# templeblock/audioSignalProcess

Measured on AMD Instinct MI355X. Metric: audio frames/sec (10 ms @16 kHz) Wiener NS, higher is better.
Workload: dtype f32

## Files before the change

audiosignalprocess_amd/csrc/ns_device.h:

```cpp
#pragma once
#include <hip/hip_runtime.h>

namespace aspns_dev {

#ifdef NS1_BUDGET
#define ASP_NS_RARE(c) (__builtin_assume(!(c)), false)
#else
#define ASP_NS_RARE(c) __builtin_expect((c), 0)
#endif

__device__ __forceinline__ float xorf(float x, uint32_t m) {
  return __uint_as_float(__float_as_uint(x) ^ m);
}

__device__ __forceinline__ void wave_lds_fence() {
  __builtin_amdgcn_fence(__ATOMIC_RELEASE, "wavefront");
  __builtin_amdgcn_wave_barrier();
  __builtin_amdgcn_fence(__ATOMIC_ACQUIRE, "wavefront");
}

template <int CTRL>
__device__ __forceinline__ float dpp_move(float v) {
  return __int_as_float(__builtin_amdgcn_update_dpp(0, __float_as_int(v), CTRL, 0xF, 0xF, true));
}
// ... 223 lines not shown
  __device__ __forceinline__ float get(int k) const { return k == 0 ? a.x : k == 1 ? a.y : k == 2 ? b.x : k == 3 ? b.y : t; }
};
__device__ __forceinline__ F5 operator+(const F5& x, const F5& y) { return F5(x.a + y.a, x.b + y.b, x.t + y.t); }
__device__ __forceinline__ F5 operator-(const F5& x, const F5& y) { return F5(x.a - y.a, x.b - y.b, x.t - y.t); }
__device__ __forceinline__ F5 operator*(const F5& x, const F5& y) { return F5(x.a * y.a, x.b * y.b, x.t * y.t); }
__device__ __forceinline__ F5 operator*(float c, const F5& y) { return F5(c) * y; }
__device__ __forceinline__ F5 operator*(const F5& x, float c) { return x * F5(c); }
__device__ __forceinline__ F5 operator+(const F5& x, float c) { return x + F5(c); }
__device__ __forceinline__ F5 operator-(const F5& x, float c) { return x - F5(c); }
__device__ __forceinline__ F5 operator-(float c, const F5& y) { return F5(c) - y; }
__device__ __forceinline__ F5 operator-(const F5& x) { return F5(-x.a, -x.b, -x.t); }
__device__ __forceinline__ F5 fma5(const F5& x, const F5& y, const F5& z) {
  return F5(__builtin_elementwise_fma(x.a, y.a, z.a), __builtin_elementwise_fma(x.b, y.b, z.b),
            __builtin_fmaf(x.t, y.t, z.t));
}
__device__ __forceinline__ F5 abs5(const F5& x) {
  return F5(f32x2{fabsf(x.a.x), fabsf(x.a.y)}, f32x2{fabsf(x.b.x), fabsf(x.b.y)}, fabsf(x.t));
}
#define ASP_F5_CMP(name, op)                                                        \
  __device__ __forceinline__ B5 name(const F5& x, const F5& y) {                    \
    B5 r;                                                                           \
    r.v[0] = x.a.x op y.a.x; r.v[1] = x.a.y op y.a.y; r.v[2] = x.b.x op y.b.x;      \
    r.v[3] = x.b.y op y.b.y; r.v[4] = x.t op y.t;                                   \
    return r;                                                                       \
  }
ASP_F5_CMP(gt5, >)
ASP_F5_CMP(lt5, <)
#undef ASP_F5_CMP
__device__ __forceinline__ F5 sel5(const B5& c, const F5& x, const F5& y) {
  return F5(f32x2{c.v[0] ? x.a.x : y.a.x, c.v[1] ? x.a.y : y.a.y},
            f32x2{c.v[2] ? x.b.x : y.b.x, c.v[3] ? x.b.y : y.b.y}, c.v[4] ? x.t : y.t);
}
__device__ __forceinline__ F5 div_by_uniform5(const F5& a, float d, float rd) {
  const F5 q0 = a * rd;
  const F5 r = fma5(F5(-d), q0, a);
  return fma5(r, F5(rd), q0);
}
__device__ __forceinline__ F5 fdiv5v(const F5& n, const F5& d) {
  return F5(fdiv2(n.a, d.a), fdiv2(n.b, d.b), fdiv(n.t, d.t));
}

__device__ __forceinline__ double log_lean_f64(float x) {
  const int xb = __float_as_int(x);
  int e = ((xb >> 23) & 0xff) - 127;
  float mf = __int_as_float((xb & 0x007fffff) | 0x3f800000);
  const bool big = mf > 1.41421356f;
  mf = big ? mf * 0.5f : mf;
  e += big ? 1 : 0;
  const float ff = mf - 1.0f;
  const float gf = mf + 1.0f;
  const double g = (double)mf + 1.0;
  const double c = (double)__builtin_amdgcn_rcpf(gf);
  const double f = (double)ff;
  const double s0 = f * c;
  const double d = __builtin_fma(g, c, -1.0);
  double s = __builtin_fma(-s0, d, s0);
  s = __builtin_fma(s0 * d, d, s);
  const double z = s * s;
  double p = 2.0 / 21.0;
  p = __builtin_fma(p, z, 2.0 / 19.0);
  p = __builtin_fma(p, z, 2.0 / 17.0);
  p = __builtin_fma(p, z, 2.0 / 15.0);
  p = __builtin_fma(p, z, 2.0 / 13.0);
  p = __builtin_fma(p, z, 2.0 / 11.0);
  p = __builtin_fma(p, z, 2.0 / 9.0);
  p = __builtin_fma(p, z, 2.0 / 7.0);
  p = __builtin_fma(p, z, 2.0 / 5.0);
  p = __builtin_fma(p, z, 2.0 / 3.0);
  const double lm = __builtin_fma(s * z, p, s + s);
  const double ed = (double)e;
  const double ln2_hi = 0x1.62e42fefa38p-1;
  const double ln2_lo = 0x1.ef35793c7673p-45;
  return __builtin_fma(ed, ln2_hi, __builtin_fma(ed, ln2_lo, lm));
}

__device__ __forceinline__ bool f64_rounds_safely_to_f32(double y) {
  const unsigned lo = (unsigned)__double2loint(y) & 0x1fffffffu;
  return ((lo - 0x0ffffe00u) > 0x400u);
}
__device__ __forceinline__ bool f64_lo_rounds_unsafely(unsigned lo) { return ((lo << 3) - 0x7ffff000u) <= 0x2000u; }
__device__ __forceinline__ bool f64_rounds_unsafely_to_f32(double y) {
  return f64_lo_rounds_unsafely((unsigned)__double2loint(y));
}

__device__ __forceinline__ double exp_lean_f64(float xf, const double* __restrict__ t64) {
  const double x = (double)xf;
  const double kd = __builtin_rint(x * 0x1.71547652b82fep+6);
  const int k = (int)kd;
  double r = __builtin_fma(-kd, 0x1.62e42ff000000p-7, x);
  r = __builtin_fma(-kd, -0x1.718432a1b0e26p-41, r);
  double q = 1.0 / 120.0;
  q = __builtin_fma(q, r, 1.0 / 24.0);
  q = __builtin_fma(q, r, 1.0 / 6.0);
  q = __builtin_fma(q, r, 0.5);
  const double p = __builtin_fma(q, r * r, r);
  const double T = t64[k & 63];
  return __builtin_amdgcn_ldexp(__builtin_fma(T, p, T), k >> 6);
}

__device__ __forceinline__ float exp_f32_via_f64(float x, const double* __restrict__ t64) {
  const bool in_range = fabsf(x) <= 87.0f;
  const double y = exp_lean_f64(in_range ? x : 0.0f, t64);
  const bool ok = in_range && f64_rounds_safely_to_f32(y);
  float r = (float)y;
  if (ASP_NS_RARE(!ok)) r = (float)exp((double)x);
  return r;
}

__device__ __forceinline__ float tanh_f32_via_f64(float a, const double* __restrict__ t64) {
  const float ax = fabsf(a);
  const bool finite_ok = ax <= 40.0f;
  const double ad = (double)ax;
  const double a2 = ad * ad;
  double sr = 0x1.664f4882c10fap-6;
  sr = __builtin_fma(sr, a2, -0x1.ba1ba1ba1ba1cp-5);
  sr = __builtin_fma(sr, a2, 0x1.1111111111111p-3);
  sr = __builtin_fma(sr, a2, -0x1.5555555555555p-2);
  const double t_small = __builtin_fma(ad * a2, sr, ad);
  const double u = exp_lean_f64(finite_ok ? -2.0f * ax : 0.0f, t64);
  const double num = 1.0 - u, den = 1.0 + u;
  double rc = (double)__builtin_amdgcn_rcpf((float)den);
  rc = __builtin_fma(__builtin_fma(-den, rc, 1.0), rc, rc);
  rc = __builtin_fma(__builtin_fma(-den, rc, 1.0), rc, rc);
  double qv = num * rc;
  qv = __builtin_fma(__builtin_fma(-qv, den, num), rc, qv);
  const double t = ax < 0.03125f ? t_small : qv;
  const bool ok = finite_ok && f64_rounds_safely_to_f32(t);
  float r = __builtin_copysignf((float)t, a);
  if (ASP_NS_RARE(!ok)) r = (float)tanh((double)a);
  return r;
}

__device__ __forceinline__ float tanh_f32_via_f64_wave(float a, const double* __restrict__ t64) {
  const float ax = fabsf(a);
  const unsigned long long far = __builtin_amdgcn_ballot_w64(!(ax <= 40.0f));
  const double u = exp_lean_f64(-2.0f * ax, t64);
  const double num = 1.0 - u, den = 1.0 + u;
  double rc = (double)__builtin_amdgcn_rcpf((float)den);
  rc = __builtin_fma(__builtin_fma(-den, rc, 1.0), rc, rc);
  double t = num * rc;
  t = __builtin_fma(__builtin_fma(-t, den, num), rc, t);
  const bool small = ax < 0.03125f;
  if (ASP_NS_RARE(__builtin_amdgcn_ballot_w64(small) != 0)) {
    const double ad = (double)ax;
    const double a2 = ad * ad;
    double sr = 0x1.664f4882c10fap-6;
    sr = __builtin_fma(sr, a2, -0x1.ba1ba1ba1ba1cp-5);
    sr = __builtin_fma(sr, a2, 0x1.1111111111111p-3);
    sr = __builtin_fma(sr, a2, -0x1.5555555555555p-2);
    const double t_small = __builtin_fma(ad * a2, sr, ad);
    t = small ? t_small : t;
  }
  const unsigned long long bad = far | __builtin_amdgcn_ballot_w64(f64_rounds_unsafely_to_f32(t));
  float r = __builtin_copysignf((float)t, a);
  if (ASP_NS_RARE(bad != 0)) r = (float)tanh((double)a);
  return r;
}

__device__ __forceinline__ float fsqrt(float x) {
  const float r = __builtin_amdgcn_rsqf(x);
  float g = x * r;
  float h = 0.5f * r;
  const float e = __builtin_fmaf(-h, g, 0.5f);
  g = __builtin_fmaf(g, e, g);
  h = __builtin_fmaf(h, e, h);
  const float d = __builtin_fmaf(-g, g, x);
// ... 16 lines not shown
constexpr unsigned kLogOff = 0x3f328000u;
__device__ __forceinline__ unsigned log_reduced_bits_mad(int k, unsigned ix) {
  unsigned z;
  asm("v_mad_i32_i24 %0, %1, %2, %3" : "=v"(z) : "v"(k), "s"(0xff800000u), "v"(ix));
  return z;
}
template <bool MAD = false>
__device__ __forceinline__ double log_tab_f64(float x, const double2* __restrict__ tab) {
  const unsigned ix = __float_as_uint(x);
  const unsigned tmp = ix - kLogOff;
  const int i = (tmp >> 16) & 127;
  const int k = (int)tmp >> 23;
  const double z = (double)__uint_as_float(MAD ? log_reduced_bits_mad(k, ix) : ix - (tmp & 0xff800000u));
  const double2 t = tab[i];
  const double r = __builtin_fma(z, t.x, -1.0);
  const double kd = (double)k;
  double p = -1.0 / 6.0;
  p = __builtin_fma(p, r, 1.0 / 5.0);
  p = __builtin_fma(p, r, -1.0 / 4.0);
  p = __builtin_fma(p, r, 1.0 / 3.0);
  p = __builtin_fma(p, r, -0.5);
  const double hi = __builtin_fma(kd, 0x1.62e42fefa38p-1, t.y);
  const double lo = __builtin_fma(kd, 0x1.ef35793c7673p-45, __builtin_fma(r * r, p, r));
  return hi + lo;
}
__device__ __forceinline__ float log_f32_via_tab(float x, const double2* __restrict__ tab) {
  const unsigned ax = __float_as_uint(x);
  const bool normal_pos = (ax - 0x00800000u) < 0x7f000000u;
  const double y = log_tab_f64(normal_pos ? x : 1.0f, tab);
  const bool ok = normal_pos && f64_rounds_safely_to_f32(y);
  float r = (float)y;
  if (__builtin_expect(!ok, 0)) r = (float)log((double)x);
  return r;
}

__device__ __attribute__((noinline)) float log_f32_slow(float x) { return (float)log((double)x); }
__device__ __attribute__((noinline)) float exp_f32_slow(float x) { return (float)exp((double)x); }
__device__ __attribute__((noinline)) float sqrt_f32_slow(float x) { return sqrtf(x); }

template <int N, bool MAD = false>
__device__ __forceinline__ void log_f32_via_tab_n(const float (&x)[N], float (&out)[N],
                                                  const double2* __restrict__ tab) {
  unsigned bad = 0;
#pragma unroll
  for (int k = 0; k < N; ++k) {
    const unsigned ax = __float_as_uint(x[k]);
    const unsigned normal_pos = (ax - 0x00800000u) < 0x7f000000u ? 1u : 0u;
    const double y = log_tab_f64<MAD>(x[k], tab);
    bad |= (normal_pos ^ 1u) | (f64_rounds_safely_to_f32(y) ? 0u : 1u);
    out[k] = (float)y;
  }
  if (ASP_NS_RARE(bad != 0)) {
#pragma unroll
    for (int k = 0; k < N; ++k) out[k] = log_f32_slow(x[k]);
  }
}

template <int N>
__device__ __forceinline__ void exp_f32_via_f64_n(const float (&x)[N], float (&out)[N],
                                                  const double* __restrict__ t64) {
  unsigned bad = 0;
#pragma unroll
  for (int k = 0; k < N; ++k) {
    const unsigned in_range = fabsf(x[k]) <= 87.0f ? 1u : 0u;
    const double y = exp_lean_f64(x[k], t64);
    bad |= (in_range ^ 1u) | (f64_rounds_safely_to_f32(y) ? 0u : 1u);
    out[k] = (float)y;
  }
  if (ASP_NS_RARE(bad != 0)) {
#pragma unroll
    for (int k = 0; k < N; ++k) out[k] = exp_f32_slow(x[k]);
  }
}

__device__ __forceinline__ unsigned long long lanes_not_positive_normal(float x) {
  unsigned long long m;
  asm("v_cmp_class_f32_e64 %0, %1, %2" : "=s"(m) : "v"(x), "s"(0x3ffu & ~0x100u));
  return m;
}
template <int N>
__device__ __forceinline__ void log_f32_via_tab_n_wave(const float (&x)[N], float (&out)[N],
                                                       const double2* __restrict__ tab) {
  unsigned long long bad = 0;
#pragma unroll
  for (int k = 0; k < N; ++k) {
    bad |= lanes_not_positive_normal(x[k]);
    const double y = log_tab_f64<true>(x[k], tab);
    bad |= __builtin_amdgcn_ballot_w64(f64_rounds_unsafely_to_f32(y));
    out[k] = (float)y;
  }
  if (ASP_NS_RARE(bad != 0)) {
#pragma unroll
    for (int k = 0; k < N; ++k) out[k] = log_f32_slow(x[k]);
  }
}

template <int N>
__device__ __forceinline__ void exp_f32_via_f64_n_wave(const float (&x)[N], float (&out)[N],
                                                       const double* __restrict__ t64) {
  unsigned long long bad = 0;
#pragma unroll
  for (int k = 0; k < N; ++k) {
    bad |= __builtin_amdgcn_ballot_w64(!(fabsf(x[k]) <= 87.0f));
    const double y = exp_lean_f64(x[k], t64);
    bad |= __builtin_amdgcn_ballot_w64(f64_rounds_unsafely_to_f32(y));
    out[k] = (float)y;
  }
  if (ASP_NS_RARE(bad != 0)) {
#pragma unroll
    for (int k = 0; k < N; ++k) out[k] = exp_f32_slow(x[k]);
  }
}

template <int N>
__device__ __forceinline__ void fsqrt_n(const float (&x)[N], float (&out)[N]) {
  unsigned bad = 0;
#pragma unroll
  for (int k = 0; k < N; ++k) {
    const float xv = x[k];
    const float r = __builtin_amdgcn_rsqf(xv);
    float g = xv * r;
    float h = 0.5f * r;
    const float e = __builtin_fmaf(-h, g, 0.5f);
    g = __builtin_fmaf(g, e, g);
    h = __builtin_fmaf(h, e, h);
    const float d = __builtin_fmaf(-g, g, xv);
    g = __builtin_fmaf(d, h, g);
    out[k] = (xv == 0.0f || xv == __builtin_inff()) ? xv : g;
    bad |= (xv < 0x1p-100f && xv > 0.0f) ? 1u : 0u;
  }
  if (ASP_NS_RARE(bad != 0)) {
#pragma unroll
    for (int k = 0; k < N; ++k)
      if (x[k] < 0x1p-100f && x[k] > 0.0f) out[k] = sqrt_f32_slow(x[k]);
  }
}

template <int N>
__device__ __forceinline__ void fsqrt_n_wave(const float (&x)[N], float (&out)[N]) {
  unsigned long long tiny = 0;
  unsigned long long passes = 0;
#pragma unroll
  for (int k = 0; k < N; ++k) {
    const float xv = x[k];
    const float r = __builtin_amdgcn_rsqf(xv);
    const float g = xv * r;
    const float h = 0.5f * r;
    const float d = __builtin_fmaf(-g, g, xv);
    out[k] = __builtin_fmaf(d, h, g);
    passes |= __builtin_amdgcn_ballot_w64(!(fabsf(out[k]) < __builtin_inff()));
    tiny |= __builtin_amdgcn_ballot_w64(xv < 0x1p-100f);
  }
  if (ASP_NS_RARE(passes != 0)) {
#pragma unroll
    for (int k = 0; k < N; ++k)
      out[k] = (x[k] == 0.0f || x[k] == __builtin_inff()) ? x[k] : (x[k] < 0.0f ? __builtin_nanf("") : out[k]);
  }
  if (ASP_NS_RARE(tiny != 0)) {
    unsigned bad = 0;
#pragma unroll
    for (int k = 0; k < N; ++k) bad |= (x[k] < 0x1p-100f && x[k] > 0.0f) ? 1u : 0u;
    if (bad != 0) {
#pragma unroll
      for (int k = 0; k < N; ++k)
        if (x[k] < 0x1p-100f && x[k] > 0.0f) out[k] = sqrt_f32_slow(x[k]);
    }
  }
}
__device__ __forceinline__ float fsqrt_wave(float x) {
  const float xs[1] = {x};
  float out[1];
  fsqrt_n_wave<1>(xs, out);
  return out[0];
}


__device__ __forceinline__ double exp_lean_f64d(double x, const double* __restrict__ t64) {
  const double kd = __builtin_rint(x * 0x1.71547652b82fep+6);
  const int k = (int)kd;
  double r = __builtin_fma(-kd, 0x1.62e42ff000000p-7, x);
  r = __builtin_fma(-kd, -0x1.718432a1b0e26p-41, r);
  double q = 1.0 / 120.0;
  q = __builtin_fma(q, r, 1.0 / 24.0);
  q = __builtin_fma(q, r, 1.0 / 6.0);
  q = __builtin_fma(q, r, 0.5);
  const double p = __builtin_fma(q, r * r, r);
  const double T = t64[k & 63];
  return __builtin_amdgcn_ldexp(__builtin_fma(T, p, T), k >> 6);
}

// ... 51 lines not shown
```

audiosignalprocess_amd/csrc/ns_kernels1.hip:

```cpp
#include <hip/hip_runtime.h>

#include <type_traits>

#include "handoff.h"
#include "ns_device.h"
#include "ns_layout.h"
#include "ns_pair_fft.h"
#include "ns_step.h"

namespace {
using namespace asphandoff;
using namespace aspns_dev;
using namespace aspns_pair;

__device__ __forceinline__ unsigned long long ns_cu_tag() {
  const unsigned hw = __builtin_amdgcn_s_getreg((7 << 11) | (8 << 6) | 4);
  const unsigned xcc = __builtin_amdgcn_s_getreg((3 << 11) | (0 << 6) | 20);
  return (unsigned long long)((xcc << 8) | hw);
}

constexpr int NS3 = 3;

template <typename V>
__device__ __forceinline__ V ns_in_vgpr(V x) {
// ... 236 lines not shown
    flow_j = blockIdx.y * fa.walk;
    flow_end = flow_j + fa.walk < fa.steps ? flow_j + fa.walk : fa.steps;
    flow_slot = ((unsigned)fa.slot0 + flow_j) % (unsigned)fa.ring;
  } else {
    NS_STAMP(0)
  }
  __shared__ __align__(16) float2 lds[4][130];
  __shared__ __align__(16) float tabs[3 * 64 * 4 + 32 * 4 * 2];
  __shared__ __align__(16) float wins[kAnal];
  __shared__ __align__(16) double exp2s[64];
  __shared__ __align__(16) double2 logts[128];
  __shared__ __align__(16) float imgs[FLOW ? 4 : 1][FLOW ? kImgDwords : 4];
  constexpr bool DEFER = FLOW && !DIAG;
  constexpr int kPendSteps = 8, kPendLanes = 3 * kPendSteps;
  __shared__ __align__(16) float pends[DEFER ? 4 : 1][DEFER ? kPendLanes : 1];
  const int tid = threadIdx.x;
  const float4* tab_src = tid < 192 ? reinterpret_cast<const float4*>(&T->tw[0][0][0]) + tid
                                    : reinterpret_cast<const float4*>(&T->spl[0][0][0]) + (tid - 192);
  const float4 tab_v = *tab_src;
  const float4 win_v = reinterpret_cast<const float4*>(T->window)[tid & 63];
  const double exp2_v = T->exp2_64[tid & 63];
  const double2 logt_v = reinterpret_cast<const double2*>(T->logtab)[tid & 127];
  const int lane = tid & 63;
  const int diagbits = T->diag[lane];
  const int wv = __builtin_amdgcn_readfirstlane(tid >> 6);
  float2* tile = lds[wv];
  const int lam = lane >> 1, h = lane & 1;
  const int g = lam >> 4, q = lam & 15;
  const int binA = q + 64 * g + 16 * h;
  const uint32_t gmask = g ? 0x80000000u : 0u;
  const int stream_raw = blockIdx.x * 4 + wv;
  bool wave_live = stream_raw < num_streams;
  const int stream = wave_live ? stream_raw : num_streams - 1;
  [[maybe_unused]] int list_stream = 0;
  if constexpr (LIST) {
    const int left = la.counts[stream] - la.frame0;
    flow_end = left < 0 ? 0u : (left > kListMaxSteps ? (unsigned)kListMaxSteps : (unsigned)left);
    wave_live = wave_live && flow_end != 0u;
    list_stream = la.streams[stream];
  }
  const int state_ix = LIST ? list_stream : stream;
  float* __restrict__ st = state + (size_t)state_ix * kStreamDwords;
  int32_t* __restrict__ hist = hist_all + (size_t)state_ix * kHistDwords;
  const StateAcc<FLOW> sa(st, FLOW ? imgs[wv] : nullptr);
  float* outj = out;
  auto diag_flush_steps = [&]() __attribute__((always_inline)) {
    if constexpr (DIAG) {
      unsigned* const counts = reinterpret_cast<unsigned*>(diag_buf);
      if (dg.mode == 2 && ns_cold(lane) == 0) {
        atomicAdd(counts + 2 * stream, diag_steps & 0xffffu);
        atomicAdd(counts + 2 * stream + 1, diag_steps >> 16);
      }
    }
  };

  lds_f32* const pend = (lds_f32*)pends[DEFER ? wv : 0];
  auto hist_flush = [&]() __attribute__((always_inline)) {
    if constexpr (DEFER) {
      const int lane_c = ns_cold(lane);
      lds_sync1();
      if (lane_c < kPendLanes) {
        const float fv = pend[lane_c];
        pend[lane_c] = -1.f;
        const int f = lane_c % 3;
        const float bw = f == 1 ? 0.05f : 0.1f, rbw = f == 1 ? 1.0f / 0.05f : 1.0f / 0.1f;
        const float lim = f == 1 ? kHist * 0.05f : kHist * 0.1f;
        if ((fv < lim) && (fv >= 0.0f))
          atomicAdd(&hist[f * kHistStride + (int)div_by_uniform(fv, bw, rbw)], 1);
      }
      lds_sync1();
    }
  };

  float sv;
  constexpr bool ROW_IMG = FLOW && !DIAG;
  const ScalarRow<ROW_IMG> srow(imgs[FLOW ? wv : 0]);
#define SC_I(k) __builtin_amdgcn_readlane(__float_as_int(sv), (k))
#define SC_F(k) srow.template f<(k)>(sv)
#define SC_SET_I(k, val) sv = writelane_bits<(k)>(sv, (int)(val))
#define SC_SET_F(k, val) srow.template set<(k)>(sv, (val))
  static_assert(S_COUNTER1 == S_COUNTER0 + 1 && S_COUNTER2 == S_COUNTER0 + 2, "the three counters: consecutive lanes");
  float4 s4;
  float2 carryA, carryB;
  float4 s4in = make_float4(0.f, 0.f, 0.f, 0.f);
  const size_t frame_uni = (size_t)stream * kBlockL;
  auto flow_load_in = [&](unsigned slot) __attribute__((always_inline)) {
    const int lane_c = ns_cold(lane);
    const unsigned frame_lane = 4u * (unsigned)((lane_c < 24 ? 24 : lane_c) - 24);
    const float* base = IO16 ? reinterpret_cast<const float*>(reinterpret_cast<const short*>(in + (size_t)slot * fa.per) + frame_uni)
                             : in + (size_t)slot * fa.per + frame_uni;
    s4in = load_frame4<IO16>(base, frame_lane);
  };
  auto flow_head = [&](auto head_c) __attribute__((always_inline)) {
    [[maybe_unused]] constexpr int ns_body_tag = decltype(head_c)::value;
    NS_STAMP(0)
    outj = out + (size_t)flow_slot * fa.per;
    const int lane_c = ns_cold(lane);
    s4 = s4in;
    if (lane_c < 24) s4 = sa.ld4(kOffAnaHist, 4 * lane_c);
    const int q2_c = lane_c & 30;
    carryA = sa.ld2(kOffSynt, q2_c + 32 * (lane_c & 1));
    carryB = sa.ld2(kOffSynt, q2_c + 64);
  };
  [[maybe_unused]] float4 img_v[FLOW ? kImgVec4 : 1];
  if constexpr (FLOW) {
    if (!LIST || wave_live) flow_load_in(flow_slot);
    if constexpr (!LIST)
      if (wave_live) wave_live = handoff_wait(fa.hand, fa.want + flow_j, stream, lane);
    if (wave_live) sa.image_request(lane, img_v);
  } else {
    sv = st[kOffScalars + lane];
    float* hbuf = st + kOffAnaHist;
    if (!IO16) {
      const float* src = lane < 24 ? hbuf + 4 * lane : in + (size_t)stream * kBlockL + 4 * (lane - 24);
      s4 = *reinterpret_cast<const float4*>(src);
    } else {
      const int lh = lane < 24 ? lane : 23, li = lane < 24 ? 24 : lane;
      const float4 ha = *reinterpret_cast<const float4*>(hbuf + 4 * lh);
      const short* in16 = reinterpret_cast<const short*>(in) + (size_t)stream * kBlockL + 4 * (li - 24);
      const short4 a = *reinterpret_cast<const short4*>(in16);
      const bool hsel = lane < 24;
      s4.x = hsel ? ha.x : (float)a.x;
      s4.y = hsel ? ha.y : (float)a.y;
      s4.z = hsel ? ha.z : (float)a.z;
      s4.w = hsel ? ha.w : (float)a.w;
    }
    carryA = *reinterpret_cast<const float2*>(st + kOffSynt + 2 * q + 32 * h);
    carryB = *reinterpret_cast<const float2*>(st + kOffSynt + 2 * q + 64);
  }

  reinterpret_cast<float4*>(tabs)[tid] = tab_v;
  if (tid < 64) exp2s[tid] = exp2_v;
  if (tid < 128) logts[tid] = logt_v;
  if (tid >= 192) reinterpret_cast<float4*>(wins)[tid - 192] = win_v;
  if constexpr (FLOW) {
    if (wave_live) sa.image_fill(lane, img_v);
  }
  if constexpr (DEFER) {
    if (lane < kPendLanes) pends[wv][lane] = -1.f;
  }
  __syncthreads();
  if (!wave_live) return;
  if constexpr (FLOW) {
    sv = sa.ld1(kOffScalars, lane);
    flow_head(std::integral_constant<int, 3>{});
  }
  const float* tws = tabs;
  const float* spls = tabs + 3 * 64 * 4;
  const PairFftLane fl = pair_fft_lane(lane, diagbits);

#define LOADV(dst, f)                                                                          \
  {                                                                                            \
    const float2 v2_ = sa.ld2(kOffVec + (f)*kVecStride, 2 * lane);                             \
    dst[0] = v2_.x; dst[1] = v2_.y;                                                            \
  }
#define LOADT(dst, f) dst[2] = SC_F(S_TAIL0 + (f));
#define LOAD3(dst, f) LOADV(dst, f) LOADT(dst, f)
#define STORE3(f, srcv)                                                                        \
  {                                                                                            \
    sa.st2(kOffVec + (f)*kVecStride, 2 * lane, srcv[0], srcv[1]);                              \
    SC_SET_F(S_TAIL0 + (f), srcv[2]);                                                          \
  }
#define STORE3_HOT(f, srcv)                                                                    \
  {                                                                                            \
    sa.st2(kOffVec + (f)*kVecStride, 2 * lane, srcv[0], srcv[1]);                              \
    if constexpr (!ROW_IMG) SC_SET_F(S_TAIL0 + (f), srcv[2]);                                  \
  }
#define NS_NEXT_FRAME()                                                                        \
  if constexpr (FLOW) {                                                                        \
    if constexpr (LIST) flow_slot = flow_slot + 1u;  \
    else flow_slot = flow_slot + 1u == (unsigned)fa.ring ? 0u : flow_slot + 1u;                \
    if (flow_j + 1u < flow_end) flow_load_in(flow_slot);                                       \
  }
#define NS_STREAM_DONE(head_tag)                                                               \
  if constexpr (FLOW) {                                                                        \
    [[maybe_unused]] constexpr int ns_body_tag = head_tag;  \
    const bool walk_done_ = flow_j + 1u >= flow_end;                                           \
    if (walk_done_) {                                                                          \
      NS_BUDGET_ASIDE()                                                                        \
      const int lane_w_ = ns_cold(lane);                                                       \
      srow.store_owned(lane_w_, sv);                                                           \
      hist_flush();       \
      if constexpr (!DEFER) lds_sync1();                                                       \
      sa.image_write_back(lane_w_);                                                            \
      handoff_drain();                                                                         \
    }                                                                                          \
    NS_STAMP(16)                                                                               \
    if (walk_done_) {                                                                          \
      NS_BUDGET_ASIDE()                                                                        \
      diag_flush_steps();                                                                      \
      if (!LIST && lane == 0) handoff_publish(fa.hand.seq + stream, fa.want + flow_j);         \
      return;                                                                                  \
    }                                                                                          \
    ++flow_j;                                                                                  \
    lds_sync1();                                                                               \
    NS_BUDGET_BACK(16)                                                                         \
    flow_head(std::integral_constant<int, head_tag>{});                                        \
    continue;                                                                                  \
  } else {                                                                                     \
    diag_flush_steps();                                                                        \
    return;                                                                                    \
  }

  constexpr bool CARRY = FLOW;
  [[maybe_unused]] f32x2 carry_stsa = {0.f, 0.f};
  [[maybe_unused]] float carry_stsa_tail = 0.f;
  [[maybe_unused]] bool carry_ok = false;
  constexpr bool RCPQ = FLOW && !DIAG;
  [[maybe_unused]] f32x2 rcpq = {0.f, 0.f};
  [[maybe_unused]] float rcpq_tail = 0.f;
  [[maybe_unused]] bool rcpq_ok = false;
  for (;;) {
    NS_BUDGET_BACK(0)
    float LQ[3][NS3], DEN[3][NS3], quant[NS3];
    float smooth[NS3], noisePrev[NS3], magnPrevA[NS3], logLrt[NS3], avgPause[NS3];


    const float4 w4 = *reinterpret_cast<const float4*>(wins + 4 * lane);
    const float wx0 = w4.x * s4.x, wx1 = w4.y * s4.y, wx2 = w4.z * s4.z, wx3 = w4.w * s4.w;
    float epart = wx0 * wx0;
    epart += wx1 * wx1;
    epart += wx2 * wx2;
    epart += wx3 * wx3;
    const float energy1 = wave_sum_bcast(epart);

    {
      const int lane_c = ns_cold(lane);
      if (lane_c >= 40) sa.st4(kOffAnaHist, 4 * (lane_c - 40), s4);
    }

    if (energy1 == 0.0f) {
      NS_BUDGET_ASIDE()
      float* y = IO16 ? reinterpret_cast<float*>(reinterpret_cast<short*>(outj) + (size_t)stream * kBlockL)
                      : outj + (size_t)stream * kBlockL;
      NS_NEXT_FRAME()
      const int lane_c = ns_cold(lane);
      float2 o01 = make_float2(0.f, 0.f);
      if (lane_c < 48) o01 = sa.ld2(kOffSynt, 2 * lane_c);
      __builtin_amdgcn_fence(__ATOMIC_ACQ_REL, "wavefront");
      store2p<IO16>(y, 2 * lane_c, sat16p(o01.x), sat16p(o01.y));
      if (lane_c < 16) store2p<IO16>(y, 128 + 2 * lane_c, 0.f, 0.f);
      if (lane_c < 48) sa.st2(kOffSynt, 2 * lane_c, 0.f, 0.f);
      NS_STREAM_DONE(3)
    }
    NS_BUDGET_BACK(0)

    LOADV(LQ[0], V_LQ0) LOADV(LQ[1], V_LQ1) LOADV(LQ[2], V_LQ2)
    LOADV(DEN[0], V_DEN0) LOADV(DEN[1], V_DEN1) LOADV(DEN[2], V_DEN2)
    LOADV(quant, V_QUANT)
    NS_STAMP(1)
    *reinterpret_cast<float4*>(&tile[2 * lane]) = make_float4(wx0, wx1, wx2, wx3);
    lds_sync1();
    f32x2 er, ei;
    {
      f32x2 ea, eb;
// ... 505 lines not shown
        overdrive = t2[0]; denoiseBound = t2[1];
      }
      float gainv[NS3];
      float gq1[NS3], gq2[NS3], snrP[NS3];
      {
        float gd1[NS3], gd2[NS3];
#pragma unroll
        for (int k = 0; k < NS3; ++k) gd1[k] = noise[k] + 0.0001f;
        fdiv3(magn, gd1, gq1);
#pragma unroll
        for (int k = 0; k < NS3; ++k) {
          float currentEstimateStsa = 0.f;
          if (magn[k] > noise[k]) currentEstimateStsa = gq1[k] - 1.f;
          snrP[k] = NS_DD_PR_SNR * prevStsa[k] + (1.f - NS_DD_PR_SNR) * currentEstimateStsa;
          gd2[k] = overdrive + snrP[k];
        }
        fdiv3(snrP, gd2, gq2);
      }
#pragma unroll
      for (int k = 0; k < NS3; ++k) {
        float gg = fmin_raw(fmax_raw(gq2[k], denoiseBound), 1.f);
        if (startup) {
          float tmp = (initMagn[k] - overdrive * pnoise[k]);
          tmp /= (initMagn[k] + 0.0001f);
          if (tmp < denoiseBound) tmp = denoiseBound;
          if (tmp > 1.f) tmp = 1.f;
          gg *= (blockInd);
          tmp *= (NS_END_STARTUP_SHORT - blockInd);
          gg += tmp;
          gg /= (NS_END_STARTUP_SHORT);
        }
        gainv[k] = gg;
        re[k] *= gg;
        im[k] *= gg;
      }
      if constexpr (CARRY) {
        carry_stsa = f32x2{gq1[0], gq1[1]} * f32x2{gainv[0], gainv[1]};
        carry_stsa_tail = gq1[2] * gainv[2];
        carry_ok = true;
      }
      STORE3_HOT(V_SMOOTH, gainv)
      STORE3_HOT(V_NOISEPREV, noise)
      auto commit_floats = [&]() __attribute__((always_inline)) {
        if constexpr (ROW_IMG) {
          SC_SET_F(S_TAIL0 + V_LOGLRT, logLrt[2]);
          SC_SET_F(S_TAIL0 + V_AVGPAUSE, avgPause[2]);
          SC_SET_F(S_TAIL0 + V_MAGNPREV_A, magn[2]);
          SC_SET_F(S_TAIL0 + V_SMOOTH, gainv[2]);
          SC_SET_F(S_TAIL0 + V_NOISEPREV, noise[2]);
        }
        SC_SET_F(S_SIGNALENERGY, signalEnergy);
        SC_SET_F(S_SUMMAGN, sumMagn);
        if (startup) {
          SC_SET_F(S_WHITE, whiteNoiseLevel);
          SC_SET_F(S_PINKNUM, pinkNoiseNumerator);
          SC_SET_F(S_PINKEXP, pinkNoiseExp);
        }
        if (window_closed) {
          SC_SET_F(S_PMP0, pm.p0);
          SC_SET_F(S_PMP1, pm.p1);
          SC_SET_F(S_PMP3, pm.p3);
          SC_SET_F(S_PMP4, pm.p4);
          SC_SET_F(S_PMP5, pm.p5);
          SC_SET_F(S_PMP6, pm.p6);
        }
        SC_SET_F(S_FD0, fd0);
        SC_SET_F(S_FD3, fd3);
        SC_SET_F(S_FD4, fd4);
        SC_SET_F(S_FD5, fd5);
        SC_SET_F(S_FD6, fd6);
        SC_SET_F(S_PRIORSPEECHPROB, priorSpeechProb);
      };
      if constexpr (ROW_IMG) {
        if (lane == 0) commit_floats();
      }

      NS_STAMP(12)
      NS_NEXT_FRAME()
      er = f32x2{re[0], re[1]};
      ei = f32x2{im[0], im[1]};
      if (lane == 0) ei.x = re[2];
      real_split1(tile, spls, lane, er, ei, true);
      lds_sync1();
      {
        const int base = 64 * g + q + 16 * h;
        float* tf = reinterpret_cast<float*>(tile);
        tf[2 * base] = er.x;
        tf[2 * base + 1] = ei.x;
        tf[2 * base + 64] = er.y;
        tf[2 * base + 65] = ei.y;
      }
      lds_sync1();
      f32x2 tr, ti;
      {
        f32x2 ea, eb;
        cft128_passes1(tile, tws, fl, lane, ea, eb);
        radix2_tail1(ea, eb, gmask, true, tr, ti);
      }
      const float td0 = tr.x * (2.f / kAnal), td1 = ti.x * (2.f / kAnal);
      const float td2 = tr.y * (2.f / kAnal), td3s = ti.y * (2.f / kAnal);

      NS_STAMP(13)
      float factor = 1.f;
      if (gainmap == 1 && blockInd > NS_END_STARTUP_LONG) {
        float e2 = td0 * td0;
        e2 += td1 * td1;
        e2 += td2 * td2;
        e2 += td3s * td3s;
        factor = ns_gain_factor<true>(wave_sum_bcast(e2), energy1, denoiseBound, priorSpeechProb);
      }

      {
        float* y = IO16 ? reinterpret_cast<float*>(reinterpret_cast<short*>(outj) + (size_t)stream * kBlockL)
                        : outj + (size_t)stream * kBlockL;
        __builtin_amdgcn_fence(__ATOMIC_ACQ_REL, "wavefront");
        const int nA = 2 * ns_cold(binA), nB = nA + 64;
        const float2 wA = *reinterpret_cast<const float2*>(wins + nA);
        const float2 wB = *reinterpret_cast<const float2*>(wins + nB);
        const float cA0 = g == 0 ? carryA.x : 0.f, cA1 = g == 0 ? carryA.y : 0.f;
        const float cB0 = (g == 0 && h == 0) ? carryB.x : 0.f, cB1 = (g == 0 && h == 0) ? carryB.y : 0.f;
        const float oA0 = cA0 + factor * (wA.x * td0), oA1 = cA1 + factor * (wA.y * td1);
        const float oB0 = cB0 + factor * (wB.x * td2), oB1 = cB1 + factor * (wB.y * td3s);
        auto emit = [&](auto sat_c) __attribute__((always_inline)) {
          constexpr bool SAT = decltype(sat_c)::value;
          if (nA >= 160) {
            sa.st2(kOffSynt, nA - 160, oA0, oA1);
          } else {
            store2p<IO16>(y, nA, SAT ? sat16p(oA0) : oA0, SAT ? sat16p(oA1) : oA1);
          }
          if (nB >= 160) {
            sa.st2(kOffSynt, nB - 160, oB0, oB1);
          } else {
            store2p<IO16>(y, nB, SAT ? sat16p(oB0) : oB0, SAT ? sat16p(oB1) : oB1);
          }
        };
        const unsigned long long may_clip =
            (__builtin_amdgcn_ballot_w64(sat16p_may_clip(oA0)) | __builtin_amdgcn_ballot_w64(sat16p_may_clip(oA1))) |
            (__builtin_amdgcn_ballot_w64(sat16p_may_clip(oB0)) | __builtin_amdgcn_ballot_w64(sat16p_may_clip(oB1)));
        if (ASP_NS_RARE(may_clip != 0)) emit(std::true_type{});
        else emit(std::false_type{});
      }

      NS_STAMP(14)
      if constexpr (STEADY) {
        sv = addlanes_bits<(1ull << S_BLOCKIND) | (7ull << S_COUNTER0), 1ull << S_MUP3>(sv);
      } else {
        SC_SET_I(S_UPDATES, updates);
        SC_SET_I(S_COUNTER0, counter[0]);
        SC_SET_I(S_COUNTER1, counter[1]);
        SC_SET_I(S_COUNTER2, counter[2]);
        SC_SET_I(S_MUP0, mup0);
        SC_SET_I(S_MUP3, mup3);
        SC_SET_I(S_BLOCKIND, blockInd);
      }
      if constexpr (!ROW_IMG) commit_floats();
    };
    if (__builtin_expect(step_steady, 1)) step_rest(std::true_type{});
    else step_rest(std::false_type{});
    if constexpr (!FLOW) sa.st1(kOffScalars, lane, sv);
    NS_STAMP(15)
    NS_STREAM_DONE(0)
  }
#undef NS_STREAM_DONE
#undef NS_NEXT_FRAME
#undef NS_STAMP
#undef NS_BUDGET_ASIDE
#undef NS_BUDGET_BACK
#undef SC_I
#undef SC_F
#undef SC_SET_I
#undef SC_SET_F
#undef LOAD3
#undef LOADV
#undef LOADT
// ... 253 lines not shown
```

audiosignalprocess_amd/csrc/ns_pair_fft.h:

```cpp
#pragma once
#include <hip/hip_runtime.h>

#include "ns_device.h"

namespace aspns_pair {
using namespace aspns_dev;

__device__ __forceinline__ void lds_sync1() {
  __builtin_amdgcn_fence(__ATOMIC_RELEASE, "wavefront");
  __builtin_amdgcn_wave_barrier();
  __builtin_amdgcn_fence(__ATOMIC_ACQUIRE, "wavefront");
}

struct PairFftLane {
  float s;
  float kap0, kap1, kap2;
  bool h;
};
__device__ __forceinline__ PairFftLane pair_fft_lane(int lane, int diagbits) {
  PairFftLane L;
  L.h = (lane & 1) != 0;
  L.s = L.h ? -1.0f : 1.0f;
  L.kap0 = (float)(diagbits & 1);
  L.kap1 = (float)((diagbits >> 1) & 1);
  L.kap2 = (float)((diagbits >> 2) & 1);
  return L;
}

template <int ROT>
__device__ __forceinline__ f32x2 rot_add(float k, f32x2 a) {
  f32x2 kk = {k, k}, r;
  if (ROT > 0)
    asm("v_pk_fma_f32 %0, %1, %2, %2 op_sel:[0,1,0] op_sel_hi:[0,0,1] neg_lo:[0,1,0]" : "=v"(r) : "v"(kk), "v"(a));
  else
    asm("v_pk_fma_f32 %0, %1, %2, %2 op_sel:[0,1,0] op_sel_hi:[0,0,1] neg_hi:[0,1,0]" : "=v"(r) : "v"(kk), "v"(a));
  return r;
}
__device__ __forceinline__ f32x2 cmul_pk(f32x2 a, f32x2 t) {
  const f32x2 p1 = a.xx * t;
  const f32x2 p2 = a.yy * t.yx;
  f32x2 r;
  asm("v_pk_add_f32 %0, %1, %2 neg_lo:[0,1]" : "=v"(r) : "v"(p1), "v"(p2));
  return r;
}

__device__ __forceinline__ void half_bfly(f32x2 c0, f32x2 c1, f32x2 c2, f32x2 c3, const PairFftLane& L,
                                          float kap, float4 tw, f32x2& first, f32x2& second) {
  const f32x2 ss = {L.s, L.s};
  const f32x2 u = __builtin_elementwise_fma(ss, c1, c0);
  const f32x2 v = __builtin_elementwise_fma(ss, c3, c2);
  const f32x2 v2 = {L.h ? -v.y : v.x, L.h ? v.x : v.y};
  const f32x2 p = u + v2, m = u - v2;
  first = cmul_pk(rot_add<+1>(kap, p), f32x2{tw.x, tw.y});
  second = cmul_pk(rot_add<-1>(kap, m), f32x2{tw.z, tw.w});
}

__device__ __forceinline__ f32x2 ldsc(const float2* t, int i) {
  const float2 v = t[i];
  return f32x2{v.x, v.y};
}
__device__ __forceinline__ void stsc(float2* t, int i, f32x2 v) { t[i] = make_float2(v.x, v.y); }

__device__ __forceinline__ void cft128_passes1(float2* tile, const float* tws, const PairFftLane& L,
                                               int lane, f32x2& oA, f32x2& oB) {
  const int b = lane >> 1;
  const int hh = lane & 1;
  f32x2 f, s;
  {
    const int rb = (int)(__brev((unsigned)b) >> 27);
    const float4 tw = *reinterpret_cast<const float4*>(tws + (0 * 64 + lane) * 4);
    half_bfly(ldsc(tile, rb), ldsc(tile, rb + 64), ldsc(tile, rb + 32), ldsc(tile, rb + 96), L, L.kap0, tw, f, s);
    lds_sync1();
    stsc(tile, 4 * b + hh, f);
    stsc(tile, 4 * b + 2 + hh, s);
  }
  lds_sync1();
  {
    const int base = 16 * (b >> 2) + (b & 3);
    const float4 tw = *reinterpret_cast<const float4*>(tws + (1 * 64 + lane) * 4);
    half_bfly(ldsc(tile, base), ldsc(tile, base + 4), ldsc(tile, base + 8), ldsc(tile, base + 12), L, L.kap1, tw, f, s);
    lds_sync1();
    stsc(tile, base + 4 * hh, f);
    stsc(tile, base + 8 + 4 * hh, s);
  }
  lds_sync1();
  {
    const int base = 64 * (b >> 4) + (b & 15);
    const float4 tw = *reinterpret_cast<const float4*>(tws + (2 * 64 + lane) * 4);
    half_bfly(ldsc(tile, base), ldsc(tile, base + 16), ldsc(tile, base + 32), ldsc(tile, base + 48), L, L.kap2, tw, oA, oB);
  }
}

__device__ __forceinline__ float tail_combine(float v, uint32_t gmask) {
  const unsigned u = __float_as_uint(v);
  const auto r = __builtin_amdgcn_permlane32_swap(u, u, false, false);
  return __uint_as_float(r[0]) + xorf(__uint_as_float(r[1]), gmask);
}
__device__ __forceinline__ void radix2_tail1(f32x2 a, f32x2 b, uint32_t gmask, bool backward, f32x2& er, f32x2& ei) {
  const float ar = tail_combine(a.x, gmask), ai = tail_combine(a.y, gmask);
  const float br = tail_combine(b.x, gmask), bi = tail_combine(b.y, gmask);
  er = f32x2{ar, br};
  ei = backward ? f32x2{-ai, -bi} : f32x2{ai, bi};
}

__device__ __forceinline__ void real_split1(float2* tile, const float* spls, int lane, f32x2& er, f32x2& ei,
                                            bool backward) {
  const int b = lane >> 1, h = lane & 1;
  const bool hi = b >= 16;
  const int base = 64 * (b >> 4) + (b & 15) + 16 * h;
  float* tf = reinterpret_cast<float*>(tile);
  lds_sync1();
  tf[2 * base] = er.x;
  tf[2 * base + 1] = ei.x;
  tf[2 * base + 64] = er.y;
  tf[2 * base + 65] = ei.y;
  lds_sync1();
  const float sg = hi ? -1.0f : 1.0f;
  const f32x2 sgs = {sg, sg};
  const int pi0 = 2 * (128 - base);
  const f32x2 per = {tf[pi0], tf[pi0 - 64]}, pei = {tf[pi0 + 1], tf[pi0 - 63]};
  const float* wp = spls + (b * 4 + h) * 2;
  const f32x2 wr = {wp[0], wp[4]}, wi = {wp[1], wp[5]};
  const f32x2 xr = sgs * (er - per), xi = ei + pei;
  f32x2 rr, ri;
  if (!backward) {
    const f32x2 yr = wr * xr - wi * xi, yi = wr * xi + wi * xr;
    rr = __builtin_elementwise_fma(-sgs, yr, er);
    ri = ei - yi;
    if (lane == 0) {
      rr.x = er.x + ei.x;
      ri.x = er.x - ei.x;
    }
  } else {
    const f32x2 yr = wr * xr + wi * xi, yi = wr * xi - wi * xr;
    rr = __builtin_elementwise_fma(-sgs, yr, er);
    ri = yi - ei;
    if (lane == 0) {
      const float hh = 0.5f * (er.x - ei.x);
      rr.x = er.x - hh;
      ri.x = -hh;
    }
  }
  er = rr;
  ei = ri;
}

template <bool IO16>
__device__ __forceinline__ void store2p(float* y, int idx, float a, float b) {
  if (IO16) {
    short2 v;
    const float kMaxRound = 32767 - 0.5f, kMinRound = -32768 + 0.5f;
    v.x = a > 0 ? (a >= kMaxRound ? (short)32767 : (short)(a + 0.5f))
                : (a <= kMinRound ? (short)-32768 : (short)(a - 0.5f));
    v.y = b > 0 ? (b >= kMaxRound ? (short)32767 : (short)(b + 0.5f))
                : (b <= kMinRound ? (short)-32768 : (short)(b - 0.5f));
    *reinterpret_cast<short2*>(reinterpret_cast<short*>(y) + idx) = v;
  } else {
    *reinterpret_cast<float2*>(y + idx) = make_float2(a, b);
  }
}

__device__ __forceinline__ float sat16p(float x) {
  return x > 32767 ? 32767 : (x < -32768 ? -32768 : x);
}
__device__ __forceinline__ bool sat16p_may_clip(float x) { return !(fabsf(x) <= 32767.f); }

template <int K>
__device__ __forceinline__ float writelane_bits(float row, int bits) {
  int r = __float_as_int(row);
  const int u = __builtin_amdgcn_readfirstlane(bits);
  asm("v_writelane_b32 %0, %1, %2" : "+v"(r) : "s"(u), "n"(K));
  return __int_as_float(r);
}
template <int K>
__device__ __forceinline__ float setlane_vgpr(float row, float val) {
  const unsigned long long mask = 1ull << K;
  asm("v_cndmask_b32 %0, %0, %1, %2" : "+v"(row) : "v"(val), "s"(mask));
  return row;
}
template <unsigned long long MASK>
__device__ __forceinline__ float mergelanes_vgpr(float row, float val) {
  const unsigned long long mask = MASK;
  asm("v_cndmask_b32 %0, %0, %1, %2" : "+v"(row) : "v"(val), "s"(mask));
  return row;
}
template <unsigned long long UP, unsigned long long DOWN>
__device__ __forceinline__ float addlanes_bits(float row) {
  int r = __float_as_int(row);
  const unsigned long long up = UP, down = DOWN;
  asm("v_addc_co_u32_e64 %0, vcc, 0, %0, %1\n\tv_subb_co_u32_e64 %0, vcc, %0, 0, %2" : "+v"(r) : "s"(up), "s"(down) : "vcc");
  return __int_as_float(r);
}
template <int K>
__device__ __forceinline__ int lanes3_bits(int a, int b, int c) {
  return __float_as_int(writelane_bits<K + 1>(writelane_bits<K>(__int_as_float(c), a), b));
}

}
```

Baseline: 517.3 million.

## Defer rounding-safety ballots, hand-code LDS pair accesses, drop the input staging copy

The exp and log batch helpers now keep a per-lane minimum rounding margin and issue one wave ballot after the loop instead of one per element, which cuts scalar ballot work. The real_split1 LDS stores and partner/twiddle loads are rewritten as inline-asm ds_write2_b32/ds_read2_b32 with explicit offsets, so paired accesses are guaranteed to be emitted as two-address instructions. The next frame's input is now loaded straight into s4, dropping the s4in staging register, and s4 is marked dead on the last iteration to shorten its live range. The volatile asm with an explicit waitcnt may stop the compiler from scheduling around these LDS accesses.

Measured after the change: 515.2 million. Within noise of the previous version (-0.4%).

```diff
diff --git a/audiosignalprocess_amd/csrc/ns_device.h b/audiosignalprocess_amd/csrc/ns_device.h
--- a/audiosignalprocess_amd/csrc/ns_device.h
+++ b/audiosignalprocess_amd/csrc/ns_device.h
@@ -329,6 +329,10 @@
 __device__ __forceinline__ bool f64_rounds_unsafely_to_f32(double y) {
   return f64_lo_rounds_unsafely((unsigned)__double2loint(y));
 }
+__device__ __forceinline__ unsigned f64_rounding_margin(double y) {
+  return ((unsigned)__double2loint(y) << 3) - 0x7ffff000u;
+}
+__device__ __forceinline__ bool rounding_margin_unsafe(unsigned t_min) { return t_min <= 0x2000u; }
 
 __device__ __forceinline__ double exp_lean_f64(float xf, const double* __restrict__ t64) {
   const double x = (double)xf;
@@ -511,13 +515,15 @@
 __device__ __forceinline__ void log_f32_via_tab_n_wave(const float (&x)[N], float (&out)[N],
                                                        const double2* __restrict__ tab) {
   unsigned long long bad = 0;
+  unsigned t_min = 0xffffffffu;
 #pragma unroll
   for (int k = 0; k < N; ++k) {
     bad |= lanes_not_positive_normal(x[k]);
     const double y = log_tab_f64<true>(x[k], tab);
-    bad |= __builtin_amdgcn_ballot_w64(f64_rounds_unsafely_to_f32(y));
+    t_min = min(t_min, f64_rounding_margin(y));
     out[k] = (float)y;
   }
+  bad |= __builtin_amdgcn_ballot_w64(rounding_margin_unsafe(t_min));
   if (ASP_NS_RARE(bad != 0)) {
 #pragma unroll
     for (int k = 0; k < N; ++k) out[k] = log_f32_slow(x[k]);
@@ -528,13 +534,15 @@
 __device__ __forceinline__ void exp_f32_via_f64_n_wave(const float (&x)[N], float (&out)[N],
                                                        const double* __restrict__ t64) {
   unsigned long long bad = 0;
+  unsigned t_min = 0xffffffffu;
 #pragma unroll
   for (int k = 0; k < N; ++k) {
     bad |= __builtin_amdgcn_ballot_w64(!(fabsf(x[k]) <= 87.0f));
     const double y = exp_lean_f64(x[k], t64);
-    bad |= __builtin_amdgcn_ballot_w64(f64_rounds_unsafely_to_f32(y));
+    t_min = min(t_min, f64_rounding_margin(y));
     out[k] = (float)y;
   }
+  bad |= __builtin_amdgcn_ballot_w64(rounding_margin_unsafe(t_min));
   if (ASP_NS_RARE(bad != 0)) {
 #pragma unroll
     for (int k = 0; k < N; ++k) out[k] = exp_f32_slow(x[k]);
diff --git a/audiosignalprocess_amd/csrc/ns_kernels1.hip b/audiosignalprocess_amd/csrc/ns_kernels1.hip
--- a/audiosignalprocess_amd/csrc/ns_kernels1.hip
+++ b/audiosignalprocess_amd/csrc/ns_kernels1.hip
@@ -342,21 +342,22 @@
   static_assert(S_COUNTER1 == S_COUNTER0 + 1 && S_COUNTER2 == S_COUNTER0 + 2, "the three counters: consecutive lanes");
   float4 s4;
   float2 carryA, carryB;
-  float4 s4in = make_float4(0.f, 0.f, 0.f, 0.f);
   const size_t frame_uni = (size_t)stream * kBlockL;
   auto flow_load_in = [&](unsigned slot) __attribute__((always_inline)) {
     const int lane_c = ns_cold(lane);
     const unsigned frame_lane = 4u * (unsigned)((lane_c < 24 ? 24 : lane_c) - 24);
     const float* base = IO16 ? reinterpret_cast<const float*>(reinterpret_cast<const short*>(in + (size_t)slot * fa.per) + frame_uni)
                              : in + (size_t)slot * fa.per + frame_uni;
-    s4in = load_frame4<IO16>(base, frame_lane);
+    s4 = load_frame4<IO16>(base, frame_lane);
+  };
+  auto s4_dead = [&]() __attribute__((always_inline)) {
+    asm("" : "=v"(s4.x), "=v"(s4.y), "=v"(s4.z), "=v"(s4.w));
   };
   auto flow_head = [&](auto head_c) __attribute__((always_inline)) {
     [[maybe_unused]] constexpr int ns_body_tag = decltype(head_c)::value;
     NS_STAMP(0)
     outj = out + (size_t)flow_slot * fa.per;
     const int lane_c = ns_cold(lane);
-    s4 = s4in;
     if (lane_c < 24) s4 = sa.ld4(kOffAnaHist, 4 * lane_c);
     const int q2_c = lane_c & 30;
     carryA = sa.ld2(kOffSynt, q2_c + 32 * (lane_c & 1));
@@ -431,6 +432,7 @@
     if constexpr (LIST) flow_slot = flow_slot + 1u;  \
     else flow_slot = flow_slot + 1u == (unsigned)fa.ring ? 0u : flow_slot + 1u;                \
     if (flow_j + 1u < flow_end) flow_load_in(flow_slot);                                       \
+    else s4_dead();                        \
   }
 #define NS_STREAM_DONE(head_tag)                                                               \
   if constexpr (FLOW) {                                                                        \
@@ -1102,14 +1104,7 @@
       if (lane == 0) ei.x = re[2];
       real_split1(tile, spls, lane, er, ei, true);
       lds_sync1();
-      {
-        const int base = 64 * g + q + 16 * h;
-        float* tf = reinterpret_cast<float*>(tile);
-        tf[2 * base] = er.x;
-        tf[2 * base + 1] = ei.x;
-        tf[2 * base + 64] = er.y;
-        tf[2 * base + 65] = ei.y;
-      }
+      store_slot_pairs(tile, 64 * g + q + 16 * h, er, ei);
       lds_sync1();
       f32x2 tr, ti;
       {
diff --git a/audiosignalprocess_amd/csrc/ns_pair_fft.h b/audiosignalprocess_amd/csrc/ns_pair_fft.h
--- a/audiosignalprocess_amd/csrc/ns_pair_fft.h
+++ b/audiosignalprocess_amd/csrc/ns_pair_fft.h
@@ -103,24 +103,38 @@
   ei = backward ? f32x2{-ai, -bi} : f32x2{ai, bi};
 }
 
+typedef __attribute__((address_space(3))) float lds_flt;
+__device__ __forceinline__ unsigned lds_addr(const float* p) { return (unsigned)(size_t)(const lds_flt*)p; }
+__device__ __forceinline__ void store_slot_pairs(float2* tile, int base, f32x2 er, f32x2 ei) {
+  const unsigned a = lds_addr(reinterpret_cast<const float*>(tile) + 2 * base);
+  asm volatile("ds_write2_b32 %0, %1, %2 offset1:64\n\tds_write2_b32 %0, %3, %4 offset0:1 offset1:65"
+               :
+               : "v"(a), "v"(er.x), "v"(er.y), "v"(ei.x), "v"(ei.y)
+               : "memory");
+}
+__device__ __forceinline__ void load_partner_pairs(const float2* tile, int pi0, const float* wp, f32x2& per, f32x2& pei,
+                                                   f32x2& wr, f32x2& wi) {
+  const unsigned a = lds_addr(reinterpret_cast<const float*>(tile) + (pi0 - 64)), w = lds_addr(wp);
+  asm volatile("ds_read2_b32 %0, %4 offset0:64\n\tds_read2_b32 %1, %4 offset0:65 offset1:1\n\t"
+               "ds_read2_b32 %2, %5 offset1:4\n\tds_read2_b32 %3, %5 offset0:1 offset1:5\n\t"
+               "s_waitcnt lgkmcnt(0)"
+               : "=&v"(per), "=&v"(pei), "=&v"(wr), "=&v"(wi)
+               : "v"(a), "v"(w)
+               : "memory");
+}
 __device__ __forceinline__ void real_split1(float2* tile, const float* spls, int lane, f32x2& er, f32x2& ei,
                                             bool backward) {
   const int b = lane >> 1, h = lane & 1;
   const bool hi = b >= 16;
   const int base = 64 * (b >> 4) + (b & 15) + 16 * h;
-  float* tf = reinterpret_cast<float*>(tile);
-  lds_sync1();
-  tf[2 * base] = er.x;
-  tf[2 * base + 1] = ei.x;
-  tf[2 * base + 64] = er.y;
-  tf[2 * base + 65] = ei.y;
+  lds_sync1();
+  store_slot_pairs(tile, base, er, ei);
   lds_sync1();
   const float sg = hi ? -1.0f : 1.0f;
   const f32x2 sgs = {sg, sg};
   const int pi0 = 2 * (128 - base);
-  const f32x2 per = {tf[pi0], tf[pi0 - 64]}, pei = {tf[pi0 + 1], tf[pi0 - 63]};
-  const float* wp = spls + (b * 4 + h) * 2;
-  const f32x2 wr = {wp[0], wp[4]}, wi = {wp[1], wp[5]};
+  f32x2 per, pei, wr, wi;
+  load_partner_pairs(tile, pi0, spls + (b * 4 + h) * 2, per, pei, wr, wi);
   const f32x2 xr = sgs * (er - per), xi = ei + pei;
   f32x2 rr, ri;
   if (!backward) {
```
